# LucasAlegre/morl-baselines

Measured on NVIDIA H100. Metric: envelope_q_updates_per_sec, higher is better.
Workload: dtype f32

## Files before the change

### include/morl_b200.h

```cpp
#ifndef MORL_B200_H_
#define MORL_B200_H_

#include <stddef.h>
#include <stdint.h>

#ifdef __cplusplus
extern "C" {
#endif

#define MORL_B200_VERSION 100

#if defined(__GNUC__)
#define MORL_API __attribute__((visibility("default")))
#else
#define MORL_API
#endif

#define MORL_OK 0
#define MORL_ERR_NULL (-1)
#define MORL_ERR_SHAPE (-2)
#define MORL_ERR_ALIGN (-3)
#define MORL_ERR_UNSUPPORTED (-4)
#define MORL_ERR_NO_DEVICE (-5)

// ... 113 lines not shown
                                  long long c_plane_stride, const float* c_scale, int reverse_tiles, int split_accumulators,
                                  const void* relu_bits_in, void* relu_bits_out, void* stream);
MORL_API int morl_gemm_planes_ln_f32(int fmt, const void* a_planes, long long a_plane_stride, const float* a_scale, const void* b_planes,
                                     long long b_plane_stride, const float* b_scale, int M, int N, int K, const float* bias, int layer_norm,
                                     const float* ln_gamma, const float* ln_beta, float ln_eps, float drop_p, const unsigned long long* drop_seed,
                                     const unsigned int* drop_offset, unsigned int drop_salt, float* c_f32, int ldc, void* c_planes, int ldp,
                                     long long c_plane_stride, const float* c_scale, int reverse_tiles, void* drop_bits_out, void* stream);
MORL_API int morl_philox_advance(unsigned int* offset, unsigned int inc, void* stream);
MORL_API int morl_gemm_chain_supported(int fmt, int M, int K);
MORL_API int morl_gemm_chain_f32(int fmt, int n_chains, int n_layers, const void* const* act_planes, long long act_plane_stride, const float* act_scale,
                                 const void* const* w_planes, long long w_plane_stride, const float* const* w_scales, const float* const* biases,
                                 int relu, const void* const* relu_bits_in, void* const* relu_bits_out, int M, int K, int k_first, void* stream);
MORL_API int morl_gemm_chain_pairs_f32(int n_chains, int n_layers, const float* const* u, const float* const* v, int B, int W, const void* const* acts,
                                       long long act_plane_stride, const float* act_scale, const void* const* w_planes, long long w_plane_stride,
                                       const float* const* w_scales, const float* const* biases, void* const* relu_bits_out, unsigned int store_mask,
                                       void* stream);
MORL_API int morl_debug_gemm_stats(unsigned long long* out8, int reset);
MORL_API int morl_ensemble_sample_f32(const float* out, const float* max_logvar, const float* min_logvar, const int32_t* model_idx, const float* noise,
                                      const float* obs, int rew_dim, int E, int N, int O, float* sample_out, float* var_out, float* uncertainty_out,
                                      void* stream);
#define MORL_TERM_NONE 0
#define MORL_TERM_HOPPER 1
#define MORL_TERM_HUMANOID 2
#define MORL_TERM_MOUNTAINCAR 3
#define MORL_TERM_LUNARLANDER 4
MORL_API size_t morl_dyna_commit_workspace_bytes(int N);
MORL_API int morl_dyna_commit_f32(const float* out, const float* max_logvar, const float* min_logvar, const int32_t* model_idx, const float* noise,
                                  const float* obs, const float* act, int rew_dim, int E, int N, int O, int A, int rule, float max_uncertainty,
                                  float* st_obs, float* st_next_obs, float* st_act, float* st_rew, float* st_done, int capacity, int ptr,
                                  float* next_alive, float* uncertainty_out, int32_t* counts_out, void* workspace, void* stream);
// ... 59 lines not shown
```

### morl_baselines_b200/_lib.py

```python

from __future__ import annotations

import ctypes as C
import os

HERE = os.path.dirname(os.path.abspath(__file__))
LIB_PATH = os.path.join(HERE, "csrc", "libmorl_b200.so")

DOT_UNFUSED, DOT_FMA, DOT_PAIRFMA = 0, 1, 2
MAP_TILE, MAP_BLOCK = 0, 1
ROWS_REFERENCE, ROWS_BMAJOR = 0, 1
AC_ELEMENTWISE_MIN, AC_SCALAR_MIN, AC_ARGMIN_GATHER = 0, 1, 2
MAX_D = 8
FMT_BF16X3, FMT_F16X2 = 0, 1

_vp, _i, _f, _d, _i64, _sz = C.c_void_p, C.c_int, C.c_float, C.c_double, C.c_int64, C.c_size_t

SIGNATURES = {
    "morl_version": (_i, []),
    "morl_last_error": (C.c_char_p, []),
    "morl_device_sm_count": (_i, []),
    "morl_envelope_td_f32": (_i, [_vp, _vp, _vp, _vp, _vp, _f, _i, _i, _i, _i, _i, _i, _vp, _vp, _vp, _vp]),
    "morl_greedy_td_f32": (_i, [_vp, _vp, _vp, _i, _i, _vp, _vp, _i, _i, _f, _i, _i, _i, _i, _vp, _vp, _vp]),
    "morl_critic_min_td_f32": (_i, [_vp, _i, _vp, _i, _i, _vp, _vp, _i, _i, _f, _i, _i, _i, _i, _vp, _vp, _vp]),
# ... 20 lines not shown
    "morl_front_unpack_f64": (_i, [_vp, _i, _i, _i, _i, _vp, _vp, _vp]),
    "morl_hypervolume_f64": (_i, [_vp, _vp, _i, _i, _vp, _vp, _vp]),
    "morl_corner_weights_f64": (_i, [_vp, _i, _i, _vp, _i, _vp, _vp]),
    "morl_polyak_f32": (_i, [_vp, _vp, _vp, _i, _i64, _d, _vp]),
    "morl_plane_overflow_count": (_i, [_i]),
    "morl_amax_scale_f32": (_i, [_vp, C.c_longlong, _i, _vp, _vp, _vp]),
    "morl_split_planes_multi": (_i, [_i, _vp, _i, _vp]),
    "morl_split_planes": (_i, [_i, _vp, _i, _i, _i, _i, _vp, _i, _i, C.c_longlong, _vp, _vp]),
    "morl_gemm_planes_f32": (_i, [_i, _vp, C.c_longlong, _vp, _vp, C.c_longlong, _vp, _i, _i, _i, _i, _vp, _i, _vp, _i, _vp, _i, _vp, _i, C.c_longlong,
                                  _vp, _i, _i, _vp, _vp, _vp]),
    "morl_gemm_planes_ln_f32": (_i, [_i, _vp, C.c_longlong, _vp, _vp, C.c_longlong, _vp, _i, _i, _i, _vp, _i, _vp, _vp, _f, _f, _vp, _vp, C.c_uint,
                                     _vp, _i, _vp, _i, C.c_longlong, _vp, _i, _vp, _vp]),
    "morl_philox_advance": (_i, [_vp, C.c_uint, _vp]),
    "morl_gemm_chain_supported": (_i, [_i, _i, _i]),
    "morl_gemm_chain_f32": (_i, [_i, _i, _i, _vp, C.c_longlong, _vp, _vp, C.c_longlong, _vp, _vp, _i, _vp, _vp, _i, _i, _i, _vp]),
    "morl_gemm_chain_pairs_f32": (_i, [_i, _i, _vp, _vp, _i, _i, _vp, C.c_longlong, _vp, _vp, C.c_longlong, _vp, _vp, _vp, C.c_uint, _vp]),
    "morl_debug_gemm_stats": (_i, [_vp, _i]),
    "morl_ensemble_sample_f32": (_i, [_vp, _vp, _vp, _vp, _vp, _vp, _i, _i, _i, _i, _vp, _vp, _vp, _vp]),
    "morl_dyna_commit_workspace_bytes": (_sz, [_i]),
    "morl_dyna_commit_f32": (_i, [_vp, _vp, _vp, _vp, _vp, _vp, _vp, _i, _i, _i, _i, _i, _i, _f, _vp, _vp, _vp, _vp, _vp, _i, _i, _vp, _vp, _vp, _vp, _vp]),
    "morl_qhead_envelope_supported": (_i, [_i, _i, _i, _i, _i, _i]),
    "morl_qhead_gemm_supported": (_i, [_i, _i, _i, _i]),
    "morl_qhead_gemm_f32": (_i, [_i, _vp, C.c_longlong, _vp, _vp, C.c_longlong, _vp, _vp, _i, _i, _i, _i, _vp, _vp]),
    "morl_qhead_envelope_td_f32": (_i, [_i, _vp, _vp, C.c_longlong, _vp, _vp, _vp, _vp, C.c_longlong, _vp, _vp, _vp, _vp, _i, _vp, _vp, _vp, _f, _i, _i,
                                        _i, _i, _i, _i, _i, _vp, _vp, _vp, _vp, _vp, _vp]),
    "morl_pairs_relu_split_planes": (_i, [_i, _vp, _vp, _i, _i, _i, _vp, C.c_longlong, _vp, _vp, _vp]),
    "morl_pairs_product_split_planes": (_i, [_i, _vp, _vp, _i, _i, _i, _vp, C.c_longlong, _vp, _vp]),
    "morl_gemm_mn_workspace_bytes": (_sz, [_i, _i, _i]),
    "morl_gemm_planes_mn_f32": (_i, [_i, _vp, C.c_longlong, _i, _i, _vp, _vp, C.c_longlong, _i, _i, _vp, _i, _i, _vp, _i, _vp, _vp, _vp]),
    "morl_colsum_planes": (_i, [_i, _vp, C.c_longlong, _vp, _i, _i, _i, _vp, _vp, _vp]),
    "morl_pairs_grad_reduce_planes": (_i, [_i, _vp, C.c_longlong, _vp, _i, _i, _i, _vp, _vp, _vp, _vp]),
# ... 50 lines not shown
```

### morl_baselines_b200/csrc/gemm_planes.cu

```cuda
#include <cuda.h>
#include <cuda_bf16.h>
#include <cuda_fp16.h>
#include <stdlib.h>
#include <string.h>

#include "common.cuh"
#include "gemm_tc.cuh"

namespace morl {

constexpr int kGemmBM = 128;
constexpr int kGemmThreads = 384;
constexpr int kGemmConsumerRegs = 232, kGemmProducerRegs = 40;
constexpr int kGemmBoxN = 32;

__device__ unsigned int g_plane_overflow;


__device__ __forceinline__ void note_overflow(float amax) {
    if (amax > 65504.f) atomicAdd(&g_plane_overflow, 1u);
}

#define MORL_DISPATCH_FMT(F_, ...)                                                         \
    switch (F_) {                                                                          \
// ... 617 lines not shown
    static constexpr uint32_t kKBlock = P * kGemmBM * kRowB;
    static constexpr uint32_t kPlaneKB = kGemmBM * kRowB;
    static constexpr uint32_t kAct = 8 * kKBlock;
    static constexpr uint32_t kBStage = P * 256 * kRowB;
    static constexpr uint32_t kOffB = kAct;
    static constexpr uint32_t kOffBias = kOffB + kStages * kBStage;
    static constexpr uint32_t kOffBar = kOffBias + 1024;
    static constexpr uint32_t kBytes = kOffBar + 256 + 1024;
    static_assert(kBytes <= 232448, "dynamic shared memory of one CTA on sm_90 (227 KB)");
};

struct alignas(64) ResChainMaps {
    CUtensorMap A[2];
    CUtensorMap B[kChainMaxJobs];
    CUtensorMap C[kChainMaxJobs];
};

struct ResChainArgs {
    int M, K, k_first, n_chains, n_layers;
    const float* bias[kChainMaxJobs];
    const float* b_scale[kChainMaxJobs];
    uint32_t* bits_out[kChainMaxJobs];
    const uint32_t* bits_in[kChainMaxJobs];
    const float* a_scale;
    int relu;
    uint32_t store;
    const float* u[2];
    const float* v[2];
    int W;
    unsigned long long* stats;
};

__device__ __forceinline__ void mma_unit_resident(float (&acc)[128], uint32_t act, const KSmem& s, Ring& ring, int n_kblk, int wg, int lane,
                                                  long long* wait_cycles) {
    using F = PlaneFmt<MORL_FMT_F16X2>;
    using R = ResPlan;
    constexpr uint32_t b_plane = 256u * R::kRowB;
    const uint32_t a_wg = act + (uint32_t)wg * 64u * R::kRowB;
    uint32_t prev = 0;
    for (int kb = 0; kb < n_kblk; ++kb) {
        const long long c0 = wait_cycles ? clock64() : 0;
        g_mbar_wait(&s.full[ring.stage], ring.phase);
        if (wait_cycles) *wait_cycles += clock64() - c0;
        wgmma_fence();
// ... 6 lines not shown
                const uint64_t ad = make_desc_k<R::kRowB>(a0 + F::pa(t) * R::kPlaneKB + ks * 32);
                const uint64_t bd = make_desc_k<R::kRowB>(b0 + F::pb(t) * b_plane + ks * 32);
                Wgmma<256>::template mma<MORL_FMT_F16X2, 0, 0>(acc, ad, bd, (kb | ks | t) != 0 ? 1u : 0u);
            }
        }
        wgmma_commit();
        if (kb > 0) {
            wgmma_wait<1>();
            if (lane == 0) g_mbar_arrive(&s.empty[prev]);
        }
        prev = ring.stage;
        ring.advance();
    }
    wgmma_wait<0>();
    if (n_kblk > 0 && lane == 0) g_mbar_arrive(&s.empty[prev]);
}

__device__ __forceinline__ uint8_t* res_chunk(uint8_t* act, int kb, int row, int q) {
    return act + (uint32_t)kb * ResPlan::kKBlock + (uint32_t)row * ResPlan::kRowB + (uint32_t)((q ^ ((row >> 1) & 3)) << 4);
}

__global__ void __launch_bounds__(kGemmThreads, 1)
gemm_chain_resident_kernel(const __grid_constant__ ResChainMaps maps, const ResChainArgs g) {
    using F = PlaneFmt<MORL_FMT_F16X2>;
    using R = ResPlan;
    constexpr int P = R::P, BN = 256;
    extern __shared__ uint8_t gsmem_raw[];
    uint8_t* sm = align_1k(gsmem_raw);
    uint8_t* act = sm;
    KSmem s;
// ... 50 lines not shown
                                }
                                g_mbar_expect_tx(act_full, (uint32_t)n_kblk_first * R::kKBlock);
                                for (int k = 0; k < n_kblk_first; ++k) tma_load_3d(act + k * R::kKBlock, &maps.A[c], act_full, k * R::BK, row0, 0);
                                ++n_in;
                            }
                            const long long c0 = g.stats ? clock64() : 0;
                            g_mbar_wait(&s.empty[ring.stage], ring.phase ^ 1u);
                            if (g.stats) w_empty += clock64() - c0;
                            uint64_t* full = &s.full[ring.stage];
                            g_mbar_expect_tx(full, R::kBStage);
                            uint8_t* bs = s.b + ring.stage * R::kBStage;
                            for (int p = 0; p < P; ++p) tma_load_3d(bs + (uint32_t)p * 256u * R::kRowB, &maps.B[job], full, kb * R::BK, 0, p);
                            ring.advance();
                        }
                    }
                }
            if (g.stats) atomicAdd(&g.stats[2], (unsigned long long)w_empty);
        }
    } else {
        warpgroup_reg_inc<kGemmConsumerRegs>();
        const int wg = warp >> 2, wr = warp & 3;
        const int l4 = lane & 3, lr = lane >> 2;
        const int trow = wg * 64 + wr * 16;
        const float s_act = ld_scale(g.a_scale);
        const uint32_t act_s = g_smem_u32(act);
        float amax = 0.f;
        float acc[128];
        Ring ring((uint32_t)R::kStages);
        long long w_full = 0, busy = 0, w_act = 0;
        const long long t_begin = g.stats ? clock64() : 0;
        uint32_t n_in = 0;
        for (int ti = 0; ti < n_ti; ++ti)
            for (int c = 0; c < g.n_chains; ++c) {
                const int row0 = tile_row(ti, c);
                if (row0 < 0) continue;
                if (pairs) {
                    if (lane == 0) asm volatile("cp.async.bulk.wait_group.read 0;" ::: "memory");
                    __syncwarp();
                    const float* u = c ? g.u[1] : g.u[0];
                    const float* v = c ? g.v[1] : g.v[0];
#pragma unroll
                    for (int h = 0; h < 2; ++h) {
                        const int rl = trow + lr + 8 * h, row = row0 + rl;
                        const bool ok = row < g.M;
                        const int b = ok ? row / g.W : 0, j = ok ? row - b * g.W : 0;
#pragma unroll 2
                        for (int kb = 0; kb < 8; ++kb) {
                            const int col = kb * 32 + 8 * l4;
                            uint32_t o[P][4];
                            if (ok) {
                                const float4* up = reinterpret_cast<const float4*>(u + (size_t)b * BN + col);
                                const float4* vp = reinterpret_cast<const float4*>(v + (size_t)j * BN + col);
                                const float4 u0 = __ldg(up), u1 = __ldg(up + 1), v0 = __ldg(vp), v1 = __ldg(vp + 1);
                                const float x[8] = {u0.x + v0.x, u0.y + v0.y, u0.z + v0.z, u0.w + v0.w, u1.x + v1.x, u1.y + v1.y, u1.z + v1.z, u1.w + v1.w};
#pragma unroll
                                for (int t = 0; t < 4; ++t) {
                                    uint32_t w[P];
                                    const float r0 = x[2 * t] < 0.f ? 0.f : x[2 * t], r1 = x[2 * t + 1] < 0.f ? 0.f : x[2 * t + 1];
                                    F::split2(r0 * s_act, r1 * s_act, w, amax);
#pragma unroll
                                    for (int p = 0; p < P; ++p) o[p][t] = w[p];
                                }
                            } else {
#pragma unroll
                                for (int t = 0; t < 4; ++t)
#pragma unroll
                                    for (int p = 0; p < P; ++p) o[p][t] = 0u;
                            }
                            uint8_t* dst = res_chunk(act, kb, rl, l4);
#pragma unroll
                            for (int p = 0; p < P; ++p) *reinterpret_cast<uint4*>(dst + p * R::kPlaneKB) = make_uint4(o[p][0], o[p][1], o[p][2], o[p][3]);
                        }
                    }
                    asm volatile("fence.proxy.async.shared::cta;" ::: "memory");
                    bar_sync_named(2 + wg, 128);
                }
                for (int l = 0; l < g.n_layers; ++l) {
                    const int job = c * g.n_layers + l;
                    const bool last = l == g.n_layers - 1, store = (g.store >> job) & 1u;
                    reload_bias(s.bias, g.bias[job], 0, BN, s_act);
                    if (!pairs && l == 0) {
                        const long long c0 = g.stats ? clock64() : 0;
                        g_mbar_wait(act_full, n_in & 1u);
                        if (g.stats) w_act += clock64() - c0;
                    }
                    mma_unit_resident(acc, act_s, s, ring, l == 0 ? n_kblk_first : n_kblk_full, wg, lane, g.stats ? &w_full : nullptr);
                    const long long c1 = g.stats ? clock64() : 0;
                    EpiArgs e;
                    e.M = g.M; e.N = BN;
                    e.k_acc = s_act / (s_act * ld_scale(g.b_scale[job]));
                    e.c_mul = 1.0f;
                    e.bias_s = s.bias; e.relu = g.relu; e.bits_in = g.bits_in[job]; e.bits_out = g.bits_out[job]; e.bits_ld = relu_bits_words(BN);
                    e.mask = nullptr; e.ld_mask = 0; e.c_f32 = nullptr; e.ldc = 0; e.planes = 1; e.ldp = BN;
                    const bool to_tile = !last || store;
                    if (to_tile) {
                        if (lane == 0) asm volatile("cp.async.bulk.wait_group.read 0;" ::: "memory");
                        __syncwarp();
                    }
                    const int rbase = row0 + trow;
#pragma unroll
                    for (int cc = 0; cc < 8; ++cc) {
                        float a[16];
#pragma unroll
                        for (int jj = 0; jj < 16; ++jj) a[jj] = acc[16 * cc + jj];
                        float x[2][8];
                        epilogue_values<false>(a, 32 * cc, rbase, lane, e, x);
                        if (to_tile) {
#pragma unroll
                            for (int h = 0; h < 2; ++h) {
// ... 10 lines not shown
                            if (store) {
                                asm volatile("fence.proxy.async.shared::cta;" ::: "memory");
                                __syncwarp();
                                if (lane == 0) {
                                    const uint32_t src = act_s + (uint32_t)cc * R::kKBlock + (uint32_t)trow * R::kRowB;
#pragma unroll
                                    for (int p = 0; p < P; ++p)
                                        asm volatile("cp.async.bulk.tensor.3d.global.shared::cta.bulk_group [%0, {%2, %3, %4}], [%1];" ::"l"(&maps.C[job]),
                                                     "r"(src + p * R::kPlaneKB), "r"(32 * cc), "r"(rbase), "r"(p)
                                                     : "memory");
                                    asm volatile("cp.async.bulk.commit_group;" ::: "memory");
                                }
                            }
                        }
                    }
                    if (!last) {
                        asm volatile("fence.proxy.async.shared::cta;" ::: "memory");
                        bar_sync_named(2 + wg, 128);
                    } else if (!pairs) {
                        __syncwarp();
                        if (lane == 0) {
                            asm volatile("cp.async.bulk.wait_group.read 0;" ::: "memory");
                            g_mbar_arrive(act_empty);
                        }
                    }
                    if (g.stats) busy += clock64() - c1;
                }
                ++n_in;
            }
        if (g.stats && warp == 0 && lane == 0) {
            atomicAdd(&g.stats[0], (unsigned long long)w_full);
            atomicAdd(&g.stats[1], (unsigned long long)(clock64() - t_begin));
            atomicAdd(&g.stats[3], (unsigned long long)busy);
            atomicAdd(&g.stats[4], (unsigned long long)w_act);
// ... 1101 lines not shown
                            c_planes, ldp, c_plane_stride, c_scale, reverse_tiles, 0, nullptr, nullptr, &a, "morl_gemm_planes_ln_f32", stream);
}

extern "C" int morl_philox_advance(unsigned int* offset, unsigned int inc, void* stream) {
    using namespace morl;
    MORL_REQUIRE(offset, MORL_ERR_NULL, "morl_philox_advance: NULL pointer argument");
    launch_k(philox_advance_kernel, dim3(1), dim3(1), 0, static_cast<cudaStream_t>(stream), offset, inc);
    return check_launch("morl_philox_advance");
}


namespace morl {
static int launch_chain_resident(ResChainArgs& g, int n_chains, int n_layers, const void* const* in, const void* const* acts, long long act_plane_stride,
                                 const float* act_scale, const void* const* w_planes, long long w_plane_stride, const float* const* w_scales,
                                 const float* const* biases, int relu, const void* const* relu_bits_in, void* const* relu_bits_out, int M, int K,
                                 const char* name, void* stream) {
    constexpr int fmt = MORL_FMT_F16X2;
    ResChainMaps maps;
    memset(&maps, 0, sizeof(maps));
    g.M = M; g.K = K; g.n_chains = n_chains; g.n_layers = n_layers; g.a_scale = act_scale; g.relu = relu ? 1 : 0;
    for (int c = 0; c < n_chains; ++c) {
        if (!g.u[0]) {
            MORL_REQUIRE(in[c] && aligned16(in[c]), MORL_ERR_NULL, "%s: NULL or misaligned input planes (chain %d)", name, c);
            const int rc = make_plane_map(&maps.A[c], fmt, in[c], M, g.k_first, (long long)M * g.k_first, kGemmBM, ResPlan::BK);
            MORL_REQUIRE(rc == 0, MORL_ERR_NO_DEVICE, "%s: cuTensorMapEncodeTiled(A) failed (%d)", name, rc);
        }
        for (int l = 0; l < n_layers; ++l) {
            const int job = c * n_layers + l;
            const int kj = l == 0 ? g.k_first : K;
            const long long w_stride = l == 0 ? (long long)256 * g.k_first : w_plane_stride;
            MORL_REQUIRE(w_planes[job] && aligned16(w_planes[job]), MORL_ERR_NULL, "%s: NULL or misaligned weight planes (chain %d, layer %d)", name, c, l);
            int rc = make_plane_map(&maps.B[job], fmt, w_planes[job], 256, kj, w_stride, 256, ResPlan::BK, true);
            MORL_REQUIRE(rc == 0, MORL_ERR_NO_DEVICE, "%s: cuTensorMapEncodeTiled(B) failed (%d)", name, rc);
            if ((g.store >> job) & 1u) {
// ... 81 lines not shown
    const int sms = sm_count();
    const int n_tiles = (M + kGemmBM - 1) / kGemmBM;
    MORL_DISPATCH_FMT(fmt, {
        constexpr size_t smem = KPlan<kFmt>::kBytes;
        g.n_stages = KPlan<kFmt>::kStages;
        set_smem_limit_once<gemm_chain_kernel<kFmt>>(smem);
        launch_k_pdl(gemm_pdl_enabled(), gemm_chain_kernel<kFmt>, dim3(n_tiles < sms ? n_tiles : sms), dim3(kGemmThreads), smem,
                     static_cast<cudaStream_t>(stream), maps, g);
    });
    return check_launch("morl_gemm_chain_f32");
}

extern "C" int morl_gemm_chain_pairs_f32(int n_chains, int n_layers, const float* const* u, const float* const* v, int B, int W, const void* const* acts,
                                         long long act_plane_stride, const float* act_scale, const void* const* w_planes, long long w_plane_stride,
                                         const float* const* w_scales, const float* const* biases, void* const* relu_bits_out, unsigned int store_mask,
                                         void* stream) {
    using namespace morl;
    MORL_REQUIRE(u && v && w_planes, MORL_ERR_NULL, "morl_gemm_chain_pairs_f32: NULL pointer argument");
    MORL_REQUIRE(n_chains >= 1 && n_chains <= 2 && n_layers >= 1 && n_chains * n_layers <= kChainMaxJobs, MORL_ERR_SHAPE,
                 "morl_gemm_chain_pairs_f32: need 1 <= n_chains <= 2 and n_chains * n_layers <= %d (got %d x %d)", kChainMaxJobs, n_chains, n_layers);
    MORL_REQUIRE(B > 0 && W > 0 && (long long)B * W <= 0x7fffffffLL && morl_gemm_chain_supported(MORL_FMT_F16X2, B * W, 256), MORL_ERR_SHAPE,
                 "morl_gemm_chain_pairs_f32: bad shape B=%d W=%d (need B W >= 256)", B, W);
    MORL_REQUIRE(store_mask < (1u << (n_chains * n_layers)), MORL_ERR_SHAPE, "morl_gemm_chain_pairs_f32: store_mask 0x%x names jobs beyond %d x %d", store_mask,
                 n_chains, n_layers);
    MORL_REQUIRE(store_mask == 0 || acts, MORL_ERR_NULL, "morl_gemm_chain_pairs_f32: stored outputs need their planes");
    ResChainArgs g;
    memset(&g, 0, sizeof(g));
    g.k_first = 256;
    g.store = store_mask;
    g.W = W;
    const void* outs[2 * (kChainMaxJobs + 1)] = {};
    for (int c = 0; c < n_chains; ++c) {
        MORL_REQUIRE(u[c] && v[c] && aligned16(u[c]) && aligned16(v[c]), MORL_ERR_ALIGN, "morl_gemm_chain_pairs_f32: u / v of chain %d NULL or not 16-byte aligned", c);
        g.u[c] = u[c];
        g.v[c] = v[c];
        for (int l = 0; l < n_layers; ++l) outs[c * (n_layers + 1) + l + 1] = acts ? acts[c * n_layers + l] : nullptr;
    }
    return launch_chain_resident(g, n_chains, n_layers, nullptr, outs, act_plane_stride, act_scale, w_planes, w_plane_stride, w_scales, biases, 1, nullptr,
                                 relu_bits_out, B * W, 256, "morl_gemm_chain_pairs_f32", stream);
}
```

### morl_baselines_b200/multi_policy/envelope/envelope.py

```python

from __future__ import annotations

import os
from typing import List, Optional, Union

import numpy as np
import torch as th
import torch.nn as nn
import torch.optim as optim

from ... import ops
from ...tc_mlp import TCPairMlp, TCPairMlpFn
from ...common.buffer import ReplayBuffer
from ...common.fused_adam import FusedClipAdam
from ...common.morl_algorithm import MOAgent, MOPolicy
from ...common.networks import NatureCNN, get_grad_norm, layer_init, mlp, polyak_update
from ...common.prioritized_buffer import PrioritizedReplayBuffer
from ...common.utils import linearly_decaying_value
from ...common.weights import equally_spaced_weights, random_weights

_FUSED_HEAD = os.environ.get("MORL_FUSED_HEAD", "1") != "0"
_PRE_REFRESH = os.environ.get("MORL_PRE_REFRESH", "1") == "1"
_HEAD_REVERSE = os.environ.get("MORL_HEAD_REVERSE", "1") == "1"
_DEFER_TREE = os.environ.get("MORL_DEFER_TREE", "1") != "0"
# ... 316 lines not shown
                                                   share_weights_with=self._tc_on, trainable=True, split_acc=split)
                if getattr(self, "_planes_fresh", False):
                    self._planes_fresh = False
                else:
                    TCPairMlp.refresh_many([self._tc_on, self._tc_tg], transposed_of=[self._tc_train] if self._tc_train is not None else [])
                early_q = None
                if _THREE_STREAMS and self._tc_train is not None:
                    main, side3 = th.cuda.current_stream(), s["side_stream3"]
                    side3.wait_stream(main)
                    with th.cuda.stream(side3):
                        dp_ = self._dp
                        ws_ = wset if dp_ is None else wset[dp_["rank"] * dp_["w_loc"] : (dp_["rank"] + 1) * dp_["w_loc"]]
                        early_q = self._tc_train.forward_pairs(obs, ws_)
                fused_head = self.envelope and _FUSED_HEAD and self.tensor_core_accumulators != "split" and self._tc_on.head_operands() is not None \
                    and ops.qhead_envelope_supported(self._tc_fmt, B, W, A, D, self._tc_on.lin[-1].in_features)
                self.fused_head_active = bool(fused_head)
                head_reverse = False
                if fused_head:
                    if self._tc_on.pair_chain_supported() and self._tc_tg.pair_chain_supported():
                        if self._nograd_chain is None:
                            self._nograd_chain = TCPairMlp.make_pair_chain([self._tc_on, self._tc_tg])
                        u_on, v_on = self._tc_on.layer1_uv(nobs, wset)
                        u_tg, v_tg = self._tc_tg.layer1_uv(nobs, wset)
                        self._nograd_chain([u_on, u_tg], [v_on, v_tg])
                        h_on, h_tg = self._tc_on.h[-1], self._tc_tg.h[-1]
                        head_reverse = _HEAD_REVERSE
                    elif self._tc_on.chain_supported() and self._tc_tg.chain_supported():
                        if self._nograd_chain is None:
                            self._nograd_chain = TCPairMlp.make_chain([self._tc_on, self._tc_tg])
                        self._tc_on.layer1(nobs, wset)
                        self._tc_tg.layer1(nobs, wset)
                        self._nograd_chain()
                        h_on, h_tg = self._tc_on.h[-1], self._tc_tg.h[-1]
# ... 431 lines not shown
```

### morl_baselines_b200/ops.py

```python

from __future__ import annotations

from typing import Optional, Tuple

import torch as th

from . import _lib
from ._lib import (
    AC_ARGMIN_GATHER,
    AC_ELEMENTWISE_MIN,
    AC_SCALAR_MIN,
    DOT_FMA,
    DOT_PAIRFMA,
    DOT_UNFUSED,
    MAP_BLOCK,
    MAP_TILE,
    ROWS_BMAJOR,
    ROWS_REFERENCE,
)

launch_count = 0


def _count(n=1):
# ... 689 lines not shown
        self._keep = (flat_a, flat_w, flat_b, flat_s, flat_m, flat_i, act_scale)
        self.relu = bool(relu)
        arr = lambda ts: (C.c_void_p * len(ts))(*[None if t is None else t.data_ptr() for t in ts])
        self._pa, self._pw, self._pb, self._ps, self._pm, self._pi = arr(flat_a), arr(flat_w), arr(flat_b), arr(flat_s), arr(flat_m), arr(flat_i)
        self._a_stride, self._w_stride, self._act_scale = a0.stride(0), 256 * self.K, act_scale

    def __call__(self):
        rc = _lib.load().morl_gemm_chain_f32(self.fmt, self.n_chains, self.n_layers, self._pa, self._a_stride, _ptr(self._act_scale), self._pw, self._w_stride,
                                             self._ps, self._pb, int(self.relu), self._pi, self._pm, self.M, self.K, self.k_first, _stream())
        _lib.check(rc, "morl_gemm_chain_f32")
        _count()


class GemmChainPairs:

    def __init__(self, outs, weights, B: int, W: int, biases=None, w_scales=None, bits=None, act_scale=None):
        import ctypes as C

        self.n_chains, self.n_layers = len(outs), len(weights[0])
        self.B, self.W, self.M = int(B), int(W), int(B) * int(W)
        flat_o = [t for ch in outs for t in ch]
        flat_w = [t for ch in weights for t in ch]
        flat_b = [None] * len(flat_w) if biases is None else [t.detach() for ch in biases for t in ch]
        flat_s = [None] * len(flat_w) if w_scales is None else [t for ch in w_scales for t in ch]
        flat_m = [None] * len(flat_w) if bits is None else [t for ch in bits for t in ch]
        if len(flat_o) != len(flat_w) or any(len(w) != self.n_layers for w in weights) or any(len(o) != self.n_layers for o in outs):
            raise _lib.MorlB200Error("GemmChainPairs: every chain needs n_layers outputs (or None) and n_layers weight tensors")
        for t in flat_w:
            if fmt_of(t) != FMT_F16X2 or tuple(t.shape[1:]) != (256, 256) or not t.is_contiguous():
                raise _lib.MorlB200Error("GemmChainPairs: weight planes must be contiguous f16x2 [2, 256, 256]")
        stored = [t for t in flat_o if t is not None]
        for t in stored:
            if fmt_of(t) != FMT_F16X2 or tuple(t.shape[1:]) != (self.M, 256) or not t.is_contiguous() or not t.is_cuda:
                raise _lib.MorlB200Error(f"GemmChainPairs: output planes must be contiguous CUDA f16x2 tensors [2, {self.M}, 256]")
        if any(t.stride(0) != stored[0].stride(0) for t in stored):
            raise _lib.MorlB200Error("GemmChainPairs: output planes need one plane stride")
        for t in flat_m:
            if t is not None and (t.dtype != th.int32 or tuple(t.shape) != (self.M, relu_bits_words(256)) or not t.is_contiguous()):
                raise _lib.MorlB200Error(f"GemmChainPairs: ReLU bit masks must be contiguous int32 [{self.M}, {relu_bits_words(256)}]")
        self.store = sum(1 << i for i, t in enumerate(flat_o) if t is not None)
        self._keep = (flat_o, flat_w, flat_b, flat_s, flat_m, act_scale)
        arr = lambda ts: (C.c_void_p * len(ts))(*[None if t is None else t.data_ptr() for t in ts])
        self._po, self._pw, self._pb, self._ps, self._pm = arr(flat_o), arr(flat_w), arr(flat_b), arr(flat_s), arr(flat_m)
        self._o_stride = stored[0].stride(0) if stored else 0
        self._w_stride, self._act_scale = flat_w[0].stride(0), act_scale

    def __call__(self, us, vs):
        import ctypes as C

        if len(us) != self.n_chains or len(vs) != self.n_chains:
            raise _lib.MorlB200Error(f"GemmChainPairs: need u and v of {self.n_chains} chains")
        for u, v in zip(us, vs):
            if (u.dtype != th.float32 or v.dtype != th.float32 or tuple(u.shape) != (self.B, 256) or tuple(v.shape) != (self.W, 256)
                    or not u.is_contiguous() or not v.is_contiguous() or not u.is_cuda or not v.is_cuda):
                raise _lib.MorlB200Error(f"GemmChainPairs: u / v must be contiguous CUDA float32 [{self.B}, 256] / [{self.W}, 256]")
        pu = (C.c_void_p * self.n_chains)(*[u.data_ptr() for u in us])
        pv = (C.c_void_p * self.n_chains)(*[v.data_ptr() for v in vs])
        rc = _lib.load().morl_gemm_chain_pairs_f32(self.n_chains, self.n_layers, pu, pv, self.B, self.W, self._po, self._o_stride, _ptr(self._act_scale),
                                                   self._pw, self._w_stride, self._ps, self._pb, self._pm, self.store, _stream())
        _lib.check(rc, "morl_gemm_chain_pairs_f32")
        _count()


def qhead_gemm_supported(fmt: int, M: int, N: int, K: int) -> bool:
    return bool(_lib.load().morl_qhead_gemm_supported(int(fmt), int(M), int(N), int(K)))


def qhead_gemm(a_planes: th.Tensor, w_planes: th.Tensor, n_out: int, bias: th.Tensor, out: Optional[th.Tensor] = None, a_scale=None, w_scale=None,
               reverse_tiles: bool = False) -> th.Tensor:
    fmt = fmt_of(a_planes)
    _, M, K = a_planes.shape
    if fmt_of(w_planes) != fmt or tuple(w_planes.shape[1:]) != (32, K) or a_planes.stride(1) != K or w_planes.stride(1) != K:
        raise _lib.MorlB200Error(f"qhead_gemm: need K-major planes A [P, M, K] and W [P, 32, K] of one format (got {tuple(a_planes.shape)}, {tuple(w_planes.shape)})")
    if out is None:
# ... 173 lines not shown
```

### morl_baselines_b200/tc_mlp.py

```python

from __future__ import annotations

import os
from typing import List, Optional

import torch as th
from torch import nn

from . import ops

_SNAKE = os.environ.get("MORL_TC_SNAKE", "1") == "1"
_CHAIN = os.environ.get("MORL_GEMM_CHAIN", "1") == "1"
_CHAIN_BWD = os.environ.get("MORL_GEMM_CHAIN_BWD", "1") == "1"
_NARROW_HEAD = os.environ.get("MORL_NARROW_HEAD", "1") == "1"
_DEFAULT_FMT = ops.FMT_BF16X3 if os.environ.get("MORL_TC_FMT", "f16x2") == "bf16x3" else ops.FMT_F16X2

MAX_HIDDEN = 512
MAX_TRAIN_W = 256
ACT_SCALE = 2.0
W_TARGET_EXP = 14
G_TARGET_EXP = 2


def _pad(n: int, m: int) -> int:
    return (n + m - 1) // m * m


class TCPairMlp:

# ... 28 lines not shown
            raise ops._lib.MorlB200Error("TCPairMlp: unsupported network (Linear/ReLU stack with hidden widths that are multiples of 64 (f16x2) or "
                                         f"32 (bf16x3) and <= {MAX_HIDDEN}, output layer <= 256 wide)")
        dev = self.lin[0].weight.device
        M = n_obs * n_w
        scaled = fmt == ops.FMT_F16X2
        self.h = [ops.empty_planes(fmt, M, l.out_features, dev) for l in self.lin[:-1]]
        self.s_act = ops.scale_tensor(ACT_SCALE, dev) if scaled else None
        if share_weights_with is not None:
            if share_weights_with.fmt != fmt:
                raise ops._lib.MorlB200Error("TCPairMlp: plans sharing weight planes must use the same operand format")
            self.wp, self.s_w = share_weights_with.wp, share_weights_with.s_w
        else:
            self.wp = [ops.empty_planes(fmt, _pad(l.out_features, 32), l.in_features, dev) for l in self.lin[1:]]
            self.s_w = [ops.scale_tensor(1.0, dev) if scaled else None for _ in self.lin[1:]]
        self.q = th.empty((M, self.lin[-1].out_features), device=dev, dtype=th.float32)
        self._chain = self._gchain = self._gbufs = None
        self.trainable = trainable
        if trainable:
            if n_w > MAX_TRAIN_W:
                raise ops._lib.MorlB200Error(f"TCPairMlp backward supports at most {MAX_TRAIN_W} weight vectors per minibatch")
            out = self.lin[-1].out_features
            self.ld_last = _pad(out, 64)
            hid = max(l.out_features for l in self.lin[:-1])
            self.g_last = ops.empty_planes(fmt, M, self.ld_last, dev)
            self.g = [ops.empty_planes(fmt, M, hid, dev) for _ in range(2)]
            self.hbits = [ops.empty_relu_bits(M, dev, l.out_features) for l in self.lin[:-1]]
            self.s_g = ops.scale_tensor(1.0, dev) if scaled else None
            self.ws_amax = th.zeros(2, device=dev, dtype=th.int32)
            self.wtp = []
            for k, l in enumerate(self.lin[1:], start=1):
                kdim = self.ld_last if k == len(self.lin) - 1 else l.out_features
# ... 30 lines not shown
                raise ops._lib.MorlB200Error("TCPairMlp.refresh_many: mixed operand formats")
            if id(p.wp) not in seen:
                seen.add(id(p.wp))
                jobs += p._weight_jobs()
        for p in transposed_of:
            jobs += p._transposed_jobs()
            p._wt_fresh = True
        for i in range(0, len(jobs), 16):
            ops.split_planes_multi(jobs[i:i + 16], fmt)

    @th.no_grad()
    def forward_pairs(self, feats: th.Tensor, wset: th.Tensor) -> th.Tensor:
        first = self.lin[0]
        if feats.shape[1] != self.feat_dim or first.in_features != self.feat_dim + wset.shape[1]:
            raise ops._lib.MorlB200Error(f"TCPairMlp: feats {tuple(feats.shape)} / wset {tuple(wset.shape)} do not match the first layer ({first.in_features} inputs)")
        a = self.forward_hidden(feats, wset, _checked=True)
        n = len(self.lin)
        last = self.lin[-1]
        wp_last = self.wp[n - 2]
        if _NARROW_HEAD and not self.split_acc and wp_last.shape[1] == 32 and ops.qhead_gemm_supported(self.fmt, a.shape[1], last.out_features, a.shape[2]):
            return ops.qhead_gemm(a, wp_last, last.out_features, last.bias.detach(), out=self.q, a_scale=self.s_act, w_scale=self.s_w[n - 2],
                                  reverse_tiles=_SNAKE and bool((n - 1) & 1))
        q, _ = ops.gemm_planes(a, wp_last, last.out_features, bias=last.bias, relu=False, out_f32=True, c_f32=self.q,
                               reverse_tiles=_SNAKE and bool((n - 1) & 1), a_scale=self.s_act, b_scale=self.s_w[n - 2], split_acc=self.split_acc)
        return q

    @th.no_grad()
    def forward_hidden(self, feats: th.Tensor, wset: th.Tensor, _checked: bool = False) -> th.Tensor:
        first = self.lin[0]
        if not _checked and (feats.shape[1] != self.feat_dim or first.in_features != self.feat_dim + wset.shape[1]):
# ... 20 lines not shown
                and ops.gemm_chain_supported(self.fmt, self.B * self.W, 256))

    def layer1(self, feats: th.Tensor, wset: th.Tensor) -> th.Tensor:
        first = self.lin[0]
        u, v = ops.pair_layer1_uv(feats, wset, first.weight.detach(), first.bias.detach())
        hb = self.hbits if self.trainable else [None] * len(self.h)
        return ops.pairs_relu_split(u, v, out=self.h[0], scale=self.s_act, relu_bits_out=hb[0])

    def layer1_uv(self, feats: th.Tensor, wset: th.Tensor):
        first = self.lin[0]
        return ops.pair_layer1_uv(feats, wset, first.weight.detach(), first.bias.detach())

    def pair_chain_supported(self) -> bool:
        return self.fmt == ops.FMT_F16X2 and self.chain_supported()

    @staticmethod
    def make_pair_chain(plans):
        specs = [p.chain_spec() for p in plans]
        outs = [[None] * (len(sp[0]) - 2) + [sp[0][-1]] for sp in specs]
        return ops.GemmChainPairs(outs, [sp[1] for sp in specs], plans[0].B, plans[0].W, [sp[2] for sp in specs], [sp[3] for sp in specs],
                                  act_scale=plans[0].s_act)

    def chain_spec(self):
        n = len(self.lin)
        hb = self.hbits if self.trainable else [None] * len(self.h)
        return (list(self.h), [self.wp[k - 1] for k in range(1, n - 1)], [self.lin[k].bias for k in range(1, n - 1)],
                [self.s_w[k - 1] for k in range(1, n - 1)], [hb[k] for k in range(1, n - 1)])

    @staticmethod
    def make_chain(plans):
        specs = [p.chain_spec() for p in plans]
        return ops.GemmChain([sp[0] for sp in specs], [sp[1] for sp in specs], [sp[2] for sp in specs], [sp[3] for sp in specs],
                             [sp[4] for sp in specs], act_scale=plans[0].s_act)

    def head_operands(self):
        last = self.lin[-1]
# ... 209 lines not shown
```

Before: 829.2.

## Fuse output Q-head GEMM into resident pair-chain kernel for forward passes

Extends the resident pair-chain kernel so the final narrow output layer (N≤32) is computed in-kernel from the last hidden activations held in shared memory, with head weights streamed through the existing TMA ring. It can also store layer-1 activations and ReLU bit masks from inside the kernel, letting the trainable forward run as a single chain launch. The envelope no-grad target path and trainable forward now use this instead of a separate head GEMM or fused envelope head. This removes the extra kernel launches and the global round-trip of the last hidden layer, at the cost of extra ring stages, more register use and more kernel complexity.

```diff
diff --git a/include/morl_b200.h b/include/morl_b200.h
--- a/include/morl_b200.h
+++ b/include/morl_b200.h
@@ -151,6 +151,8 @@
 MORL_API int morl_gemm_chain_pairs_f32(int n_chains, int n_layers, const float* const* u, const float* const* v, int B, int W, const void* const* acts,
                                        long long act_plane_stride, const float* act_scale, const void* const* w_planes, long long w_plane_stride,
                                        const float* const* w_scales, const float* const* biases, void* const* relu_bits_out, unsigned int store_mask,
+                                       void* const* h0_planes, void* const* h0_bits, const void* const* head_w, long long head_w_plane_stride,
+                                       const float* const* head_scales, const float* const* head_biases, int head_n, float* const* q_out,
                                        void* stream);
 MORL_API int morl_debug_gemm_stats(unsigned long long* out8, int reset);
 MORL_API int morl_ensemble_sample_f32(const float* out, const float* max_logvar, const float* min_logvar, const int32_t* model_idx, const float* noise,
diff --git a/morl_baselines_b200/_lib.py b/morl_baselines_b200/_lib.py
--- a/morl_baselines_b200/_lib.py
+++ b/morl_baselines_b200/_lib.py
@@ -58,7 +58,8 @@
     "morl_philox_advance": (_i, [_vp, C.c_uint, _vp]),
     "morl_gemm_chain_supported": (_i, [_i, _i, _i]),
     "morl_gemm_chain_f32": (_i, [_i, _i, _i, _vp, C.c_longlong, _vp, _vp, C.c_longlong, _vp, _vp, _i, _vp, _vp, _i, _i, _i, _vp]),
-    "morl_gemm_chain_pairs_f32": (_i, [_i, _i, _vp, _vp, _i, _i, _vp, C.c_longlong, _vp, _vp, C.c_longlong, _vp, _vp, _vp, C.c_uint, _vp]),
+    "morl_gemm_chain_pairs_f32": (_i, [_i, _i, _vp, _vp, _i, _i, _vp, C.c_longlong, _vp, _vp, C.c_longlong, _vp, _vp, _vp, C.c_uint, _vp, _vp, _vp,
+                                  C.c_longlong, _vp, _vp, _i, _vp, _vp]),
     "morl_debug_gemm_stats": (_i, [_vp, _i]),
     "morl_ensemble_sample_f32": (_i, [_vp, _vp, _vp, _vp, _vp, _vp, _i, _i, _i, _i, _vp, _vp, _vp, _vp]),
     "morl_dyna_commit_workspace_bytes": (_sz, [_i]),
diff --git a/morl_baselines_b200/csrc/gemm_planes.cu b/morl_baselines_b200/csrc/gemm_planes.cu
--- a/morl_baselines_b200/csrc/gemm_planes.cu
+++ b/morl_baselines_b200/csrc/gemm_planes.cu
@@ -655,6 +655,8 @@
     CUtensorMap A[2];
     CUtensorMap B[kChainMaxJobs];
     CUtensorMap C[kChainMaxJobs];
+    CUtensorMap Q[2];
+    CUtensorMap H0[2];
 };
 
 struct ResChainArgs {
@@ -669,6 +671,13 @@
     const float* u[2];
     const float* v[2];
     int W;
+    int store_h0;
+    uint32_t* h0_bits[2];
+    int head;
+    int q_n;
+    const float* q_bias[2];
+    const float* q_scale[2];
+    float* q_out[2];
     unsigned long long* stats;
 };
 
@@ -705,6 +714,32 @@
     }
     wgmma_wait<0>();
     if (n_kblk > 0 && lane == 0) g_mbar_arrive(&s.empty[prev]);
+}
+
+__device__ __forceinline__ void mma_head_resident(float (&acc)[16], uint32_t act, const KSmem& s, Ring& ring, int wg, int lane, long long* wait_cycles) {
+    using F = PlaneFmt<MORL_FMT_F16X2>;
+    using R = ResPlan;
+    constexpr uint32_t b_box = 32u * R::kRowB;
+    const uint32_t a_wg = act + (uint32_t)wg * 64u * R::kRowB;
+    const long long c0 = wait_cycles ? clock64() : 0;
+    g_mbar_wait(&s.full[ring.stage], ring.phase);
+    if (wait_cycles) *wait_cycles += clock64() - c0;
+    wgmma_fence();
+    const uint32_t b0 = g_smem_u32(s.b + ring.stage * R::kBStage);
+#pragma unroll
+    for (int kb = 0; kb < 256 / R::BK; ++kb)
+#pragma unroll
+        for (int ks = 0; ks < R::BK / 16; ++ks)
+#pragma unroll
+            for (int t = 0; t < F::NPROD; ++t) {
+                const uint64_t ad = make_desc_k<R::kRowB>(a_wg + (uint32_t)kb * R::kKBlock + F::pa(t) * R::kPlaneKB + ks * 32);
+                const uint64_t bd = make_desc_k<R::kRowB>(b0 + ((uint32_t)kb * R::P + F::pb(t)) * b_box + ks * 32);
+                Wgmma<32>::template mma<MORL_FMT_F16X2, 0, 0>(acc, ad, bd, (kb | ks | t) != 0 ? 1u : 0u);
+            }
+    wgmma_commit();
+    wgmma_wait<0>();
+    if (lane == 0) g_mbar_arrive(&s.empty[ring.stage]);
+    ring.advance();
 }
 
 __device__ __forceinline__ uint8_t* res_chunk(uint8_t* act, int kb, int row, int q) {
@@ -785,6 +820,18 @@
                             ring.advance();
                         }
                     }
+                    if ((g.head >> c) & 1) {
+                        const long long c0 = g.stats ? clock64() : 0;
+                        g_mbar_wait(&s.empty[ring.stage], ring.phase ^ 1u);
+                        if (g.stats) w_empty += clock64() - c0;
+                        uint64_t* full = &s.full[ring.stage];
+                        static_assert(P * 32 * 256 * 2 == R::kBStage, "the output layer's weight planes fill one ring stage");
+                        g_mbar_expect_tx(full, R::kBStage);
+                        uint8_t* bs = s.b + ring.stage * R::kBStage;
+                        for (int kb = 0; kb < 256 / R::BK; ++kb)
+                            for (int p = 0; p < P; ++p) tma_load_3d(bs + (uint32_t)(kb * P + p) * 32u * R::kRowB, &maps.Q[c], full, kb * R::BK, 0, p);
+                        ring.advance();
+                    }
                 }
             if (g.stats) atomicAdd(&g.stats[2], (unsigned long long)w_empty);
         }
@@ -810,6 +857,7 @@
                     __syncwarp();
                     const float* u = c ? g.u[1] : g.u[0];
                     const float* v = c ? g.v[1] : g.v[0];
+                    uint32_t* bits0 = c ? g.h0_bits[1] : g.h0_bits[0];
 #pragma unroll
                     for (int h = 0; h < 2; ++h) {
                         const int rl = trow + lr + 8 * h, row = row0 + rl;
@@ -819,6 +867,7 @@
                         for (int kb = 0; kb < 8; ++kb) {
                             const int col = kb * 32 + 8 * l4;
                             uint32_t o[P][4];
+                            uint32_t pos = 0;
                             if (ok) {
                                 const float4* up = reinterpret_cast<const float4*>(u + (size_t)b * BN + col);
                                 const float4* vp = reinterpret_cast<const float4*>(v + (size_t)j * BN + col);
@@ -828,6 +877,7 @@
                                 for (int t = 0; t < 4; ++t) {
                                     uint32_t w[P];
                                     const float r0 = x[2 * t] < 0.f ? 0.f : x[2 * t], r1 = x[2 * t + 1] < 0.f ? 0.f : x[2 * t + 1];
+                                    pos |= (r0 > 0.f ? 1u : 0u) << (2 * t) | (r1 > 0.f ? 1u : 0u) << (2 * t + 1);
                                     F::split2(r0 * s_act, r1 * s_act, w, amax);
 #pragma unroll
                                     for (int p = 0; p < P; ++p) o[p][t] = w[p];
@@ -841,9 +891,30 @@
                             uint8_t* dst = res_chunk(act, kb, rl, l4);
 #pragma unroll
                             for (int p = 0; p < P; ++p) *reinterpret_cast<uint4*>(dst + p * R::kPlaneKB) = make_uint4(o[p][0], o[p][1], o[p][2], o[p][3]);
+                            if (bits0) {
+                                uint32_t wbits = pos << (8 * l4);
+                                wbits |= __shfl_xor_sync(0xffffffffu, wbits, 1);
+                                wbits |= __shfl_xor_sync(0xffffffffu, wbits, 2);
+                                if (l4 == 0 && ok) bits0[(size_t)row * relu_bits_words(BN) + relu_bits_word(32 * kb)] = wbits;
+                            }
                         }
                     }
                     asm volatile("fence.proxy.async.shared::cta;" ::: "memory");
+                    if ((g.store_h0 >> c) & 1) {
+                        __syncwarp();
+                        if (lane == 0) {
+#pragma unroll 1
+                            for (int kb = 0; kb < 8; ++kb) {
+                                const uint32_t src = act_s + (uint32_t)kb * R::kKBlock + (uint32_t)trow * R::kRowB;
+#pragma unroll
+                                for (int p = 0; p < P; ++p)
+                                    asm volatile("cp.async.bulk.tensor.3d.global.shared::cta.bulk_group [%0, {%2, %3, %4}], [%1];" ::"l"(c ? &maps.H0[1] : &maps.H0[0]),
+                                                 "r"(src + p * R::kPlaneKB), "r"(32 * kb), "r"(row0 + trow), "r"(p)
+                                                 : "memory");
+                            }
+                            asm volatile("cp.async.bulk.commit_group;" ::: "memory");
+                        }
+                    }
                     bar_sync_named(2 + wg, 128);
                 }
                 for (int l = 0; l < g.n_layers; ++l) {
@@ -863,7 +934,8 @@
                     e.c_mul = 1.0f;
                     e.bias_s = s.bias; e.relu = g.relu; e.bits_in = g.bits_in[job]; e.bits_out = g.bits_out[job]; e.bits_ld = relu_bits_words(BN);
                     e.mask = nullptr; e.ld_mask = 0; e.c_f32 = nullptr; e.ldc = 0; e.planes = 1; e.ldp = BN;
-                    const bool to_tile = !last || store;
+                    const bool head = last && ((g.head >> c) & 1);
+                    const bool to_tile = !last || store || head;
                     if (to_tile) {
                         if (lane == 0) asm volatile("cp.async.bulk.wait_group.read 0;" ::: "memory");
                         __syncwarp();
@@ -904,10 +976,31 @@
                             }
                         }
                     }
-                    if (!last) {
+                    if (!last || head) {
                         asm volatile("fence.proxy.async.shared::cta;" ::: "memory");
                         bar_sync_named(2 + wg, 128);
-                    } else if (!pairs) {
+                    }
+                    if (head) {
+                        float accq[16];
+                        mma_head_resident(accq, act_s, s, ring, wg, lane, g.stats ? &w_full : nullptr);
+                        const float kq = 1.0f / (s_act * ld_scale(c ? g.q_scale[1] : g.q_scale[0]));
+                        const float* qb = c ? g.q_bias[1] : g.q_bias[0];
+                        float* qo = c ? g.q_out[1] : g.q_out[0];
+#pragma unroll
+                        for (int h = 0; h < 2; ++h) {
+                            const int row = rbase + lr + 8 * h;
+                            if (row < g.M) {
+#pragma unroll
+                                for (int q = 0; q < 4; ++q)
+#pragma unroll
+                                    for (int cq = 0; cq < 2; ++cq) {
+                                        const int col = 8 * q + 2 * l4 + cq;
+                                        if (col < g.q_n) qo[(size_t)row * g.q_n + col] = __fmaf_rn(accq[4 * q + 2 * h + cq], kq, qb ? __ldg(qb + col) : 0.f);
+                                    }
+                            }
+                        }
+                    }
+                    if (last && !pairs) {
                         __syncwarp();
                         if (lane == 0) {
                             asm volatile("cp.async.bulk.wait_group.read 0;" ::: "memory");
@@ -2039,10 +2132,23 @@
 static int launch_chain_resident(ResChainArgs& g, int n_chains, int n_layers, const void* const* in, const void* const* acts, long long act_plane_stride,
                                  const float* act_scale, const void* const* w_planes, long long w_plane_stride, const float* const* w_scales,
                                  const float* const* biases, int relu, const void* const* relu_bits_in, void* const* relu_bits_out, int M, int K,
-                                 const char* name, void* stream) {
+                                 const char* name, void* stream, const void* const* h0 = nullptr, const void* const* head_w = nullptr,
+                                 long long head_w_stride = 0) {
     constexpr int fmt = MORL_FMT_F16X2;
     ResChainMaps maps;
     memset(&maps, 0, sizeof(maps));
+    for (int c = 0; c < n_chains; ++c) {
+        if ((g.store_h0 >> c) & 1) {
+            MORL_REQUIRE(h0 && h0[c] && aligned16(h0[c]), MORL_ERR_NULL, "%s: NULL or misaligned h0 planes (chain %d)", name, c);
+            const int rc = make_plane_map(&maps.H0[c], fmt, h0[c], M, 256, act_plane_stride, 16, 32, true);
+            MORL_REQUIRE(rc == 0, MORL_ERR_NO_DEVICE, "%s: cuTensorMapEncodeTiled(h0) failed (%d)", name, rc);
+        }
+        if ((g.head >> c) & 1) {
+            MORL_REQUIRE(head_w && head_w[c] && aligned16(head_w[c]), MORL_ERR_NULL, "%s: NULL or misaligned head weight planes (chain %d)", name, c);
+            const int rc = make_plane_map(&maps.Q[c], fmt, head_w[c], 32, K, head_w_stride, 32, ResPlan::BK, true);
+            MORL_REQUIRE(rc == 0, MORL_ERR_NO_DEVICE, "%s: cuTensorMapEncodeTiled(head) failed (%d)", name, rc);
+        }
+    }
     g.M = M; g.K = K; g.n_chains = n_chains; g.n_layers = n_layers; g.a_scale = act_scale; g.relu = relu ? 1 : 0;
     for (int c = 0; c < n_chains; ++c) {
         if (!g.u[0]) {
@@ -2154,6 +2260,8 @@
 extern "C" int morl_gemm_chain_pairs_f32(int n_chains, int n_layers, const float* const* u, const float* const* v, int B, int W, const void* const* acts,
                                          long long act_plane_stride, const float* act_scale, const void* const* w_planes, long long w_plane_stride,
                                          const float* const* w_scales, const float* const* biases, void* const* relu_bits_out, unsigned int store_mask,
+                                         void* const* h0_planes, void* const* h0_bits, const void* const* head_w, long long head_w_plane_stride,
+                                         const float* const* head_scales, const float* const* head_biases, int head_n, float* const* q_out,
                                          void* stream) {
     using namespace morl;
     MORL_REQUIRE(u && v && w_planes, MORL_ERR_NULL, "morl_gemm_chain_pairs_f32: NULL pointer argument");
@@ -2170,12 +2278,28 @@
     g.store = store_mask;
     g.W = W;
     const void* outs[2 * (kChainMaxJobs + 1)] = {};
+    const void* h0[2] = {nullptr, nullptr};
     for (int c = 0; c < n_chains; ++c) {
         MORL_REQUIRE(u[c] && v[c] && aligned16(u[c]) && aligned16(v[c]), MORL_ERR_ALIGN, "morl_gemm_chain_pairs_f32: u / v of chain %d NULL or not 16-byte aligned", c);
         g.u[c] = u[c];
         g.v[c] = v[c];
         for (int l = 0; l < n_layers; ++l) outs[c * (n_layers + 1) + l + 1] = acts ? acts[c * n_layers + l] : nullptr;
-    }
+        if (h0_planes && h0_planes[c]) {
+            g.store_h0 |= 1 << c;
+            h0[c] = h0_planes[c];
+        }
+        g.h0_bits[c] = h0_bits ? static_cast<uint32_t*>(h0_bits[c]) : nullptr;
+        MORL_REQUIRE(aligned16(g.h0_bits[c]), MORL_ERR_ALIGN, "morl_gemm_chain_pairs_f32: ReLU bit masks of h0 must be 16-byte aligned (chain %d)", c);
+        if (head_w && head_w[c]) {
+            MORL_REQUIRE(head_n >= 1 && head_n <= 32, MORL_ERR_UNSUPPORTED, "morl_gemm_chain_pairs_f32: the output layer needs 1 <= N <= 32 (N=%d)", head_n);
+            MORL_REQUIRE(q_out && q_out[c] && aligned16(q_out[c]), MORL_ERR_ALIGN, "morl_gemm_chain_pairs_f32: Q of chain %d NULL or not 16-byte aligned", c);
+            g.head |= 1 << c;
+            g.q_out[c] = q_out[c];
+            g.q_scale[c] = head_scales ? head_scales[c] : nullptr;
+            g.q_bias[c] = head_biases ? head_biases[c] : nullptr;
+        }
+    }
+    g.q_n = head_n;
     return launch_chain_resident(g, n_chains, n_layers, nullptr, outs, act_plane_stride, act_scale, w_planes, w_plane_stride, w_scales, biases, 1, nullptr,
-                                 relu_bits_out, B * W, 256, "morl_gemm_chain_pairs_f32", stream);
-}
+                                 relu_bits_out, B * W, 256, "morl_gemm_chain_pairs_f32", stream, h0, head_w, head_w_plane_stride);
+}
diff --git a/morl_baselines_b200/multi_policy/envelope/envelope.py b/morl_baselines_b200/multi_policy/envelope/envelope.py
--- a/morl_baselines_b200/multi_policy/envelope/envelope.py
+++ b/morl_baselines_b200/multi_policy/envelope/envelope.py
@@ -354,9 +354,18 @@
                         early_q = self._tc_train.forward_pairs(obs, ws_)
                 fused_head = self.envelope and _FUSED_HEAD and self.tensor_core_accumulators != "split" and self._tc_on.head_operands() is not None \
                     and ops.qhead_envelope_supported(self._tc_fmt, B, W, A, D, self._tc_on.lin[-1].in_features)
+                chain_head = fused_head and self._tc_on.chain_head_supported() and self._tc_tg.chain_head_supported()
+                fused_head = fused_head and not chain_head
                 self.fused_head_active = bool(fused_head)
                 head_reverse = False
-                if fused_head:
+                if chain_head:
+                    if self._nograd_chain is None:
+                        self._nograd_chain = TCPairMlp.make_pair_chain([self._tc_on, self._tc_tg], head=True)
+                    u_on, v_on = self._tc_on.layer1_uv(nobs, wset)
+                    u_tg, v_tg = self._tc_tg.layer1_uv(nobs, wset)
+                    self._nograd_chain([u_on, u_tg], [v_on, v_tg])
+                    q_on, q_tg = self._tc_on.q.view(B, W, A, D), self._tc_tg.q.view(B, W, A, D)
+                elif fused_head:
                     if self._tc_on.pair_chain_supported() and self._tc_tg.pair_chain_supported():
                         if self._nograd_chain is None:
                             self._nograd_chain = TCPairMlp.make_pair_chain([self._tc_on, self._tc_tg])
diff --git a/morl_baselines_b200/ops.py b/morl_baselines_b200/ops.py
--- a/morl_baselines_b200/ops.py
+++ b/morl_baselines_b200/ops.py
@@ -727,11 +727,31 @@
 
 class GemmChainPairs:
 
-    def __init__(self, outs, weights, B: int, W: int, biases=None, w_scales=None, bits=None, act_scale=None):
+    def __init__(self, outs, weights, B: int, W: int, biases=None, w_scales=None, bits=None, act_scale=None, h0=None, h0_bits=None, heads=None,
+                 q_out=None):
         import ctypes as C
 
         self.n_chains, self.n_layers = len(outs), len(weights[0])
         self.B, self.W, self.M = int(B), int(W), int(B) * int(W)
+        nc = self.n_chains
+        h0 = [None] * nc if h0 is None else list(h0)
+        h0_bits = [None] * nc if h0_bits is None else list(h0_bits)
+        heads = [None] * nc if heads is None else list(heads)
+        q_out = [None] * nc if q_out is None else list(q_out)
+        if not (len(h0) == len(h0_bits) == len(heads) == len(q_out) == nc):
+            raise _lib.MorlB200Error(f"GemmChainPairs: h0 / h0_bits / heads / q_out need one entry per chain ({nc})")
+        self.head_n = 0
+        for hd, q in zip(heads, q_out):
+            if hd is None:
+                continue
+            wq, _, bq = hd
+            n = bq.numel()
+            if fmt_of(wq) != FMT_F16X2 or tuple(wq.shape[1:]) != (32, 256) or not wq.is_contiguous() or not 1 <= n <= 32 or (self.head_n and n != self.head_n):
+                raise _lib.MorlB200Error("GemmChainPairs: an output layer needs contiguous f16x2 weight planes [2, 32, 256] and 1 <= N <= 32 (one N for all chains)")
+            if not (isinstance(q, th.Tensor) and q.is_cuda and q.dtype == th.float32 and q.is_contiguous() and tuple(q.shape) == (self.M, n)
+                    and q.data_ptr() % 16 == 0):
+                raise _lib.MorlB200Error(f"GemmChainPairs: Q must be a 16-byte aligned contiguous CUDA float32 tensor [{self.M}, {n}]")
+            self.head_n = n
         flat_o = [t for ch in outs for t in ch]
         flat_w = [t for ch in weights for t in ch]
         flat_b = [None] * len(flat_w) if biases is None else [t.detach() for ch in biases for t in ch]
@@ -742,20 +762,25 @@
         for t in flat_w:
             if fmt_of(t) != FMT_F16X2 or tuple(t.shape[1:]) != (256, 256) or not t.is_contiguous():
                 raise _lib.MorlB200Error("GemmChainPairs: weight planes must be contiguous f16x2 [2, 256, 256]")
-        stored = [t for t in flat_o if t is not None]
+        stored = [t for t in flat_o + h0 if t is not None]
         for t in stored:
             if fmt_of(t) != FMT_F16X2 or tuple(t.shape[1:]) != (self.M, 256) or not t.is_contiguous() or not t.is_cuda:
                 raise _lib.MorlB200Error(f"GemmChainPairs: output planes must be contiguous CUDA f16x2 tensors [2, {self.M}, 256]")
         if any(t.stride(0) != stored[0].stride(0) for t in stored):
             raise _lib.MorlB200Error("GemmChainPairs: output planes need one plane stride")
-        for t in flat_m:
+        for t in flat_m + h0_bits:
             if t is not None and (t.dtype != th.int32 or tuple(t.shape) != (self.M, relu_bits_words(256)) or not t.is_contiguous()):
                 raise _lib.MorlB200Error(f"GemmChainPairs: ReLU bit masks must be contiguous int32 [{self.M}, {relu_bits_words(256)}]")
         self.store = sum(1 << i for i, t in enumerate(flat_o) if t is not None)
-        self._keep = (flat_o, flat_w, flat_b, flat_s, flat_m, act_scale)
+        hw = [None if hd is None else hd[0] for hd in heads]
+        hs = [None if hd is None else hd[1] for hd in heads]
+        hb = [None if hd is None else hd[2].detach() for hd in heads]
+        self._keep = (flat_o, flat_w, flat_b, flat_s, flat_m, act_scale, h0, h0_bits, hw, hs, hb, q_out)
         arr = lambda ts: (C.c_void_p * len(ts))(*[None if t is None else t.data_ptr() for t in ts])
         self._po, self._pw, self._pb, self._ps, self._pm = arr(flat_o), arr(flat_w), arr(flat_b), arr(flat_s), arr(flat_m)
+        self._ph0, self._ph0b, self._phw, self._phs, self._phb, self._pq = arr(h0), arr(h0_bits), arr(hw), arr(hs), arr(hb), arr(q_out)
         self._o_stride = stored[0].stride(0) if stored else 0
+        self._hw_stride = next((t.stride(0) for t in hw if t is not None), 0)
         self._w_stride, self._act_scale = flat_w[0].stride(0), act_scale
 
     def __call__(self, us, vs):
@@ -770,7 +795,8 @@
         pu = (C.c_void_p * self.n_chains)(*[u.data_ptr() for u in us])
         pv = (C.c_void_p * self.n_chains)(*[v.data_ptr() for v in vs])
         rc = _lib.load().morl_gemm_chain_pairs_f32(self.n_chains, self.n_layers, pu, pv, self.B, self.W, self._po, self._o_stride, _ptr(self._act_scale),
-                                                   self._pw, self._w_stride, self._ps, self._pb, self._pm, self.store, _stream())
+                                                   self._pw, self._w_stride, self._ps, self._pb, self._pm, self.store, self._ph0, self._ph0b, self._phw,
+                                                   self._hw_stride, self._phs, self._phb, self.head_n, self._pq, _stream())
         _lib.check(rc, "morl_gemm_chain_pairs_f32")
         _count()
 
diff --git a/morl_baselines_b200/tc_mlp.py b/morl_baselines_b200/tc_mlp.py
--- a/morl_baselines_b200/tc_mlp.py
+++ b/morl_baselines_b200/tc_mlp.py
@@ -13,6 +13,7 @@
 _CHAIN = os.environ.get("MORL_GEMM_CHAIN", "1") == "1"
 _CHAIN_BWD = os.environ.get("MORL_GEMM_CHAIN_BWD", "1") == "1"
 _NARROW_HEAD = os.environ.get("MORL_NARROW_HEAD", "1") == "1"
+_CHAIN_HEAD = os.environ.get("MORL_CHAIN_HEAD", "1") != "0"
 _DEFAULT_FMT = ops.FMT_BF16X3 if os.environ.get("MORL_TC_FMT", "f16x2") == "bf16x3" else ops.FMT_F16X2
 
 MAX_HIDDEN = 512
@@ -71,7 +72,7 @@
             self.wp = [ops.empty_planes(fmt, _pad(l.out_features, 32), l.in_features, dev) for l in self.lin[1:]]
             self.s_w = [ops.scale_tensor(1.0, dev) if scaled else None for _ in self.lin[1:]]
         self.q = th.empty((M, self.lin[-1].out_features), device=dev, dtype=th.float32)
-        self._chain = self._gchain = self._gbufs = None
+        self._chain = self._gchain = self._gbufs = self._head_chain = None
         self.trainable = trainable
         if trainable:
             if n_w > MAX_TRAIN_W:
@@ -132,6 +133,12 @@
         first = self.lin[0]
         if feats.shape[1] != self.feat_dim or first.in_features != self.feat_dim + wset.shape[1]:
             raise ops._lib.MorlB200Error(f"TCPairMlp: feats {tuple(feats.shape)} / wset {tuple(wset.shape)} do not match the first layer ({first.in_features} inputs)")
+        if self.trainable and self.chain_head_supported():
+            if self._head_chain is None:
+                self._head_chain = TCPairMlp.make_pair_chain([self], head=True, store_all=True)
+            u, v = self.layer1_uv(feats, wset)
+            self._head_chain([u], [v])
+            return self.q
         a = self.forward_hidden(feats, wset, _checked=True)
         n = len(self.lin)
         last = self.lin[-1]
@@ -182,12 +189,23 @@
     def pair_chain_supported(self) -> bool:
         return self.fmt == ops.FMT_F16X2 and self.chain_supported()
 
-    @staticmethod
-    def make_pair_chain(plans):
+    def chain_head_supported(self) -> bool:
+        return _CHAIN_HEAD and self.pair_chain_supported() and self.head_operands() is not None
+
+    @staticmethod
+    def make_pair_chain(plans, head: bool = False, store_all: bool = False):
         specs = [p.chain_spec() for p in plans]
-        outs = [[None] * (len(sp[0]) - 2) + [sp[0][-1]] for sp in specs]
+        if store_all:
+            outs = [sp[0][1:] for sp in specs]
+        else:
+            outs = [[None] * (len(sp[0]) - 1) if head else [None] * (len(sp[0]) - 2) + [sp[0][-1]] for sp in specs]
+        kw = {}
+        if store_all:
+            kw.update(bits=[sp[4] for sp in specs], h0=[p.h[0] for p in plans], h0_bits=[p.hbits[0] if p.trainable else None for p in plans])
+        if head:
+            kw.update(heads=[p.head_operands() for p in plans], q_out=[p.q for p in plans])
         return ops.GemmChainPairs(outs, [sp[1] for sp in specs], plans[0].B, plans[0].W, [sp[2] for sp in specs], [sp[3] for sp in specs],
-                                  act_scale=plans[0].s_act)
+                                  act_scale=plans[0].s_act, **kw)
 
     def chain_spec(self):
         n = len(self.lin)
```

Result: faster. 851.0 (median of 6 runs) (+2.6%).
